# yzhang511/multi_modal_foundation_model

Hardware: NVIDIA B200
Metric: train trials/sec fwd+bwd (higher is better)
Workload: dtype bf16

## Files before the change

multi_modal_foundation_model_b200/csrc/common.cuh:

```cuda
#pragma once
#include <cuda.h>
#include <cuda_bf16.h>
#include <cuda_runtime.h>
#include <stdint.h>
#include <stdio.h>

namespace mmfm {

typedef __nv_bfloat16 bf16;

#define MMFM_DEVINL __device__ __forceinline__

MMFM_DEVINL uint32_t smem_u32(const void* p) { return (uint32_t)__cvta_generic_to_shared(p); }

MMFM_DEVINL bool elect_one() {
  uint32_t pred = 0;
  asm volatile(
      "{\n\t.reg .pred P1;\n\t.reg .b32 R1;\n\t"
      "elect.sync R1|P1, 0xffffffff;\n\t"
      "selp.u32 %0, 1, 0, P1;\n\t}\n"
      : "=r"(pred));
  return pred != 0;
}

// ... 37 lines not shown
      : "memory");
#else
  asm volatile(
      "{\n\t.reg .pred p;\n\t"
      "mbarrier.try_wait.parity.shared::cta.b64 p, [%1], %2;\n\t"
      "selp.u32 %0, 1, 0, p;\n\t}\n"
      : "=r"(ok)
      : "r"(smem_u32(bar)), "r"(parity)
      : "memory");
#endif
  return ok != 0;
}
MMFM_DEVINL void mbar_wait(uint64_t* bar, uint32_t parity) {
  if (mbar_try_wait(bar, parity)) return;
  uint32_t n = 0;
  while (!mbar_try_wait(bar, parity)) {
    if (++n > MMFM_MBAR_SPIN_LIMIT) {
      printf("mmfm: mbarrier wait timeout block(%d,%d,%d) thread %d parity %u bar %u\n", blockIdx.x, blockIdx.y,
             blockIdx.z, threadIdx.x, parity, smem_u32(bar));
      __trap();
    }
  }
}
MMFM_DEVINL void mbar_wait_relaxed(uint64_t* bar, uint32_t parity) {
  if (mbar_try_wait(bar, parity)) return;
  uint32_t n = 0;
  while (!mbar_try_wait(bar, parity)) {
    __nanosleep(40);
    if (++n > MMFM_MBAR_SPIN_LIMIT) {
      printf("mmfm: mbarrier wait timeout block(%d,%d,%d) thread %d parity %u bar %u\n", blockIdx.x, blockIdx.y,
             blockIdx.z, threadIdx.x, parity, smem_u32(bar));
      __trap();
    }
  }
}

MMFM_DEVINL void tma_prefetch_desc(const CUtensorMap* m) {
  asm volatile("prefetch.tensormap [%0];" ::"l"(m) : "memory");
}
MMFM_DEVINL void tma_load_2d_addr(uint32_t smem_dst, const CUtensorMap* m, uint64_t* bar, int c0, int c1) {
  asm volatile(
      "cp.async.bulk.tensor.2d.shared::cluster.global.mbarrier::complete_tx::bytes [%0], [%1, {%3, %4}], [%2];"
      ::"r"(smem_dst), "l"(m), "r"(smem_u32(bar)), "r"(c0), "r"(c1)
      : "memory");
}

MMFM_DEVINL void tma_store_2d(const CUtensorMap* m, uint32_t smem_src, int c0, int c1) {
  asm volatile("cp.async.bulk.tensor.2d.global.shared::cta.bulk_group [%0, {%2, %3}], [%1];" ::"l"(m), "r"(smem_src),
               "r"(c0), "r"(c1)
               : "memory");
}
MMFM_DEVINL void tma_store_3d(const CUtensorMap* m, uint32_t smem_src, int c0, int c1, int c2) {
  asm volatile("cp.async.bulk.tensor.3d.global.shared::cta.bulk_group [%0, {%2, %3, %4}], [%1];" ::"l"(m), "r"(smem_src),
               "r"(c0), "r"(c1), "r"(c2)
               : "memory");
}
MMFM_DEVINL void bulk_commit_group() { asm volatile("cp.async.bulk.commit_group;" ::: "memory"); }
template <int N>
MMFM_DEVINL void bulk_wait_group_read() {
  asm volatile("cp.async.bulk.wait_group.read %0;" ::"n"(N) : "memory");
}
template <int N>
MMFM_DEVINL void bulk_wait_group() {
  asm volatile("cp.async.bulk.wait_group %0;" ::"n"(N) : "memory");
}

MMFM_DEVINL void tma_load_2d_mc(uint32_t smem_dst, const CUtensorMap* m, uint64_t* bar, int c0, int c1, uint16_t mask) {
  asm volatile(
      "cp.async.bulk.tensor.2d.shared::cluster.global.mbarrier::complete_tx::bytes.multicast::cluster [%0], [%1, {%3, %4}], [%2], %5;"
      ::"r"(smem_dst), "l"(m), "r"(smem_u32(bar)), "r"(c0), "r"(c1), "h"(mask)
      : "memory");
}
MMFM_DEVINL void umma_commit_mc(uint64_t* bar, uint16_t mask) {
  asm volatile("tcgen05.commit.cta_group::1.mbarrier::arrive::one.shared::cluster.multicast::cluster.b64 [%0], %1;" ::"r"(
                   smem_u32(bar)),
               "h"(mask)
               : "memory");
}
MMFM_DEVINL uint32_t cluster_ctarank() {
  uint32_t r;
  asm volatile("mov.u32 %0, %%cluster_ctarank;" : "=r"(r));
  return r;
}
MMFM_DEVINL void cluster_sync_all() {
  asm volatile("barrier.cluster.arrive.release.aligned;\n\tbarrier.cluster.wait.acquire.aligned;" ::: "memory");
}

MMFM_DEVINL void tma_prefetch_l2_2d(const CUtensorMap* m, int c0, int c1) {
  asm volatile("cp.async.bulk.prefetch.tensor.2d.L2.global.tile [%0, {%1, %2}];" ::"l"(m), "r"(c0), "r"(c1) : "memory");
}

MMFM_DEVINL void tmem_alloc(uint32_t* smem_slot, uint32_t ncols) {
  asm volatile("tcgen05.alloc.cta_group::1.sync.aligned.shared::cta.b32 [%0], %1;" ::"r"(smem_u32(smem_slot)),
               "r"(ncols)
               : "memory");
}
MMFM_DEVINL void tmem_relinquish() {
  asm volatile("tcgen05.relinquish_alloc_permit.cta_group::1.sync.aligned;" ::: "memory");
}
MMFM_DEVINL void tmem_dealloc(uint32_t taddr, uint32_t ncols) {
  asm volatile("tcgen05.dealloc.cta_group::1.sync.aligned.b32 %0, %1;" ::"r"(taddr), "r"(ncols) : "memory");
}
MMFM_DEVINL void tc_fence_before() { asm volatile("tcgen05.fence::before_thread_sync;" ::: "memory"); }
MMFM_DEVINL void tc_fence_after() { asm volatile("tcgen05.fence::after_thread_sync;" ::: "memory"); }

MMFM_DEVINL void umma_bf16(uint32_t tmem_d, uint64_t desc_a, uint64_t desc_b, uint32_t idesc, uint32_t accumulate) {
  asm volatile(
      "{\n\t.reg .pred p;\n\t"
      "setp.ne.b32 p, %4, 0;\n\t"
      "tcgen05.mma.cta_group::1.kind::f16 [%0], %1, %2, %3, p;\n\t}\n" ::"r"(tmem_d),
      "l"(desc_a), "l"(desc_b), "r"(idesc), "r"(accumulate)
      : "memory");
}
MMFM_DEVINL void umma_bf16_ts(uint32_t tmem_d, uint32_t tmem_a, uint64_t desc_b, uint32_t idesc, uint32_t accumulate) {
  asm volatile(
      "{\n\t.reg .pred p;\n\t"
      "setp.ne.b32 p, %4, 0;\n\t"
      "tcgen05.mma.cta_group::1.kind::f16 [%0], [%1], %2, %3, p;\n\t}\n" ::"r"(tmem_d),
      "r"(tmem_a), "l"(desc_b), "r"(idesc), "r"(accumulate)
      : "memory");
}
MMFM_DEVINL void umma_commit(uint64_t* bar) {
  asm volatile("tcgen05.commit.cta_group::1.mbarrier::arrive::one.shared::cluster.b64 [%0];" ::"r"(smem_u32(bar))
               : "memory");
}

MMFM_DEVINL void tmem_ld32(uint32_t taddr, uint32_t (&r)[32]) {
  asm volatile(
      "tcgen05.ld.sync.aligned.32x32b.x32.b32 "
      "{%0, %1, %2, %3, %4, %5, %6, %7, %8, %9, %10, %11, %12, %13, %14, %15, "
      "%16, %17, %18, %19, %20, %21, %22, %23, %24, %25, %26, %27, %28, %29, %30, %31}, [%32];"
      : "=r"(r[0]), "=r"(r[1]), "=r"(r[2]), "=r"(r[3]), "=r"(r[4]), "=r"(r[5]), "=r"(r[6]), "=r"(r[7]),
        "=r"(r[8]), "=r"(r[9]), "=r"(r[10]), "=r"(r[11]), "=r"(r[12]), "=r"(r[13]), "=r"(r[14]), "=r"(r[15]),
        "=r"(r[16]), "=r"(r[17]), "=r"(r[18]), "=r"(r[19]), "=r"(r[20]), "=r"(r[21]), "=r"(r[22]),
        "=r"(r[23]), "=r"(r[24]), "=r"(r[25]), "=r"(r[26]), "=r"(r[27]), "=r"(r[28]), "=r"(r[29]),
        "=r"(r[30]), "=r"(r[31])
      : "r"(taddr)
      : "memory");
}
MMFM_DEVINL void tmem_ld16(uint32_t taddr, uint32_t (&r)[16]) {
  asm volatile(
      "tcgen05.ld.sync.aligned.32x32b.x16.b32 "
      "{%0, %1, %2, %3, %4, %5, %6, %7, %8, %9, %10, %11, %12, %13, %14, %15}, [%16];"
      : "=r"(r[0]), "=r"(r[1]), "=r"(r[2]), "=r"(r[3]), "=r"(r[4]), "=r"(r[5]), "=r"(r[6]), "=r"(r[7]),
        "=r"(r[8]), "=r"(r[9]), "=r"(r[10]), "=r"(r[11]), "=r"(r[12]), "=r"(r[13]), "=r"(r[14]), "=r"(r[15])
      : "r"(taddr)
      : "memory");
}
MMFM_DEVINL void tmem_ld_wait() { asm volatile("tcgen05.wait::ld.sync.aligned;" ::: "memory"); }
MMFM_DEVINL void tmem_st16(uint32_t taddr, const uint32_t (&r)[16]) {
  asm volatile(
      "tcgen05.st.sync.aligned.32x32b.x16.b32 [%0], "
      "{%1, %2, %3, %4, %5, %6, %7, %8, %9, %10, %11, %12, %13, %14, %15, %16};" ::"r"(taddr),
      "r"(r[0]), "r"(r[1]), "r"(r[2]), "r"(r[3]), "r"(r[4]), "r"(r[5]), "r"(r[6]), "r"(r[7]), "r"(r[8]), "r"(r[9]),
      "r"(r[10]), "r"(r[11]), "r"(r[12]), "r"(r[13]), "r"(r[14]), "r"(r[15])
      : "memory");
}
MMFM_DEVINL void tmem_st8(uint32_t taddr, const uint32_t (&r)[8]) {
  asm volatile("tcgen05.st.sync.aligned.32x32b.x8.b32 [%0], {%1, %2, %3, %4, %5, %6, %7, %8};" ::"r"(taddr), "r"(r[0]),
               "r"(r[1]), "r"(r[2]), "r"(r[3]), "r"(r[4]), "r"(r[5]), "r"(r[6]), "r"(r[7])
               : "memory");
}
MMFM_DEVINL void tmem_st_wait() { asm volatile("tcgen05.wait::st.sync.aligned;" ::: "memory"); }

MMFM_DEVINL uint64_t make_smem_desc(uint32_t saddr, uint32_t lbo_bytes, uint32_t sbo_bytes, uint32_t layout) {
  uint64_t d = 0;
  d |= (uint64_t)((saddr >> 4) & 0x3FFF);
  d |= (uint64_t)((lbo_bytes >> 4) & 0x3FFF) << 16;
  d |= (uint64_t)((sbo_bytes >> 4) & 0x3FFF) << 32;
  d |= (uint64_t)1 << 46;
  d |= (uint64_t)(layout & 7) << 61;
  return d;
}
__host__ __device__ inline uint32_t make_idesc_bf16(uint32_t M, uint32_t N, uint32_t a_mn, uint32_t b_mn) {
  uint32_t d = 0;
  d |= 1u << 4;
  d |= 1u << 7;
  d |= 1u << 10;
  d |= (a_mn & 1u) << 15;
  d |= (b_mn & 1u) << 16;
  d |= ((N >> 3) & 0x3F) << 17;
  d |= ((M >> 4) & 0x1F) << 24;
  return d;
}

constexpr int kPhiloxRounds = 7;

MMFM_DEVINL void mulhilo32(uint32_t a, uint32_t b, uint32_t& hi, uint32_t& lo) {
  const unsigned long long p = (unsigned long long)a * (unsigned long long)b;
  hi = (uint32_t)(p >> 32);
  lo = (uint32_t)p;
}

MMFM_DEVINL uint4 philox4x32(uint32_t c0, uint32_t c1, uint32_t c2, uint32_t c3, uint32_t k0, uint32_t k1) {
#pragma unroll
  for (int r = 0; r < kPhiloxRounds; ++r) {
    uint32_t hi0, lo0, hi1, lo1;
    mulhilo32(0xD2511F53u, c0, hi0, lo0);
    mulhilo32(0xCD9E8D57u, c2, hi1, lo1);
    const uint32_t n0 = hi1 ^ c1 ^ k0;
    const uint32_t n2 = hi0 ^ c3 ^ k1;
    c0 = n0; c1 = lo1; c2 = n2; c3 = lo0;
    k0 += 0x9E3779B9u; k1 += 0xBB67AE85u;
  }
  return make_uint4(c0, c1, c2, c3);
}
// ... 224 lines not shown
```

multi_modal_foundation_model_b200/csrc/gemm_ts.cu:

```cuda
#include "common.cuh"
#include <stdlib.h>
#include "host_util.h"
#include "../../include/mmfm_b200.h"

#ifdef MMFM_DBG_TIMING
__device__ long long g_dbg_ts[8][64];
__device__ __forceinline__ long long dbg_now() {
  long long t;
  asm volatile("mov.u64 %0, %%globaltimer;" : "=l"(t) :: "memory");
  return t;
}
#define DBG_TS(role, slot) do { if (blockIdx.x == 5 && (slot) < 64) g_dbg_ts[role][slot] = dbg_now(); } while (0)
__device__ long long g_dbg_cta[160][2];
extern "C" int mmfm_debug_read_gemm_ts(long long* out) {
  return (int)cudaMemcpyFromSymbol(out, g_dbg_ts, sizeof(long long) * 8 * 64);
}
extern "C" int mmfm_debug_read_gemm_cta(long long* out) {
  return (int)cudaMemcpyFromSymbol(out, g_dbg_cta, sizeof(long long) * 160 * 2);
}
#else
#define DBG_TS(role, slot) do { } while (0)
#endif

namespace mmfm {

constexpr int kTsBM = 128, kTsBK = 64;
constexpr int kTsEpiWarps = 16, kTsFirstEpi = 4;
constexpr int kTsThreads = (kTsFirstEpi + kTsEpiWarps) * 32;

enum TsEpi : int {
  TS_BF16 = 0,
  TS_SOFTSIGN = 1,
  TS_F32 = 2,
  TS_RES = 3,
  TS_GELU_DG = 4,
  TS_MULAUX = 5,
  TS_DSOFTSIGN = 6,
  TS_ROWDOT = 7
};

template <int EPI>
struct TsCfg {
  static constexpr bool kF32 = EPI == TS_F32 || EPI == TS_RES;
  static constexpr bool kHasIn = EPI == TS_RES || EPI == TS_MULAUX || EPI == TS_DSOFTSIGN || EPI == TS_ROWDOT;
  static constexpr bool kTwoOut = EPI == TS_GELU_DG;
  static constexpr uint32_t kRowBytes = kF32 ? 128u : 64u;
  static constexpr uint32_t kSlice = 128u * kRowBytes;
  static constexpr uint32_t kOut = 4u * kSlice;
  static constexpr uint32_t kBuf = kOut * (kTwoOut ? 2u : 1u);
};
constexpr int kTsMaxStages = 6;
constexpr size_t kTsMaxSmem = 230400;

template <int EPI, int BN>
__global__ void __launch_bounds__(kTsThreads, 1) gemm_tn_ts_kernel(const __grid_constant__ CUtensorMap tmA,
                                                                    const __grid_constant__ CUtensorMap tmB,
                                                                    const __grid_constant__ CUtensorMap tmD,
                                                                    const __grid_constant__ CUtensorMap tmD2,
                                                                    const __grid_constant__ CUtensorMap tmIn,
                                                                    const mmfm_gemm_args p, int tiles_n, int n_tiles,
                                                                    int bstat, int nst) {
  using Cfg = TsCfg<EPI>;
  constexpr int STAGES = kTsMaxStages;
  constexpr uint32_t kABytes = kTsBM * kTsBK * 2, kBBytes = BN * kTsBK * 2;
  constexpr uint32_t kTsStageBytes = kABytes + kBBytes;
  constexpr int NU = BN / 128;
  constexpr int kTsBN = BN;
  extern __shared__ uint8_t smem_raw[];
  __shared__ __align__(8) uint64_t full_bar[STAGES], empty_bar[STAGES];
  __shared__ __align__(8) uint64_t acc_full[2], acc_empty[2], in_full[2], stg_full[2], stg_free[2], b_full;
  __shared__ uint32_t tmem_slot;

  const int warp = threadIdx.x >> 5, lane = threadIdx.x & 31;
  const int nkb = (p.K + kTsBK - 1) / kTsBK;
  if (threadIdx.x == 0) DBG_TS(7, 63);
#ifdef MMFM_DBG_TIMING
  if (threadIdx.x == 0 && blockIdx.x < 160) g_dbg_cta[blockIdx.x][0] = dbg_now();
#endif
  const uint32_t smem_base = (smem_u32(smem_raw) + 1023u) & ~1023u;
  uint8_t* smem_al = smem_raw + (smem_base - smem_u32(smem_raw));
  const uint32_t b_res = bstat ? (uint32_t)nkb * kBBytes : 0u;
  const uint32_t st_bytes = bstat ? kABytes : kTsStageBytes;
  const uint32_t ring_base = smem_base + b_res;
  const uint32_t stg_off = b_res + (uint32_t)nst * st_bytes;
  const uint32_t stg_base = smem_base + stg_off;
  uint8_t* stg_ptr = smem_al + stg_off;

  pdl_trigger();
  if (warp == 0 && lane == 0) {
    tma_prefetch_desc(&tmA);
    tma_prefetch_desc(&tmB);
    tma_prefetch_desc(&tmD);
    if (Cfg::kTwoOut) tma_prefetch_desc(&tmD2);
    if (Cfg::kHasIn) tma_prefetch_desc(&tmIn);
#pragma unroll
    for (int s = 0; s < STAGES; ++s) {
      mbar_init(&full_bar[s], 1);
      mbar_init(&empty_bar[s], 1);
    }
#pragma unroll
    for (int i = 0; i < 2; ++i) {
      mbar_init(&acc_full[i], 1);
      mbar_init(&acc_empty[i], kTsEpiWarps);
      mbar_init(&in_full[i], 1);
      mbar_init(&stg_full[i], kTsEpiWarps);
      mbar_init(&stg_free[i], 1);
    }
    mbar_init(&b_full, 1);
    fence_mbar_init();
  }
  if (warp == 1) {
    tmem_alloc(&tmem_slot, 2u * BN);
    tmem_relinquish();
  }
  tc_fence_before();
  __syncthreads();
  tc_fence_after();
  const uint32_t tmem_base = tmem_slot;
  pdl_wait();

  if (warp == 0) {
    if (elect_one()) {
      uint32_t it = 0;
      const uint32_t ns = (uint32_t)nst;
      if (bstat) {
        const int n0 = ((int)blockIdx.x % tiles_n) * kTsBN;
        mbar_arrive_expect_tx(&b_full, b_res);
        for (int kb = 0; kb < nkb; ++kb) tma_load_2d_addr(smem_base + kb * kBBytes, &tmB, &b_full, kb * kTsBK, n0);
      }
      for (int tile = blockIdx.x; tile < n_tiles; tile += gridDim.x) {
        const int m0 = (tile / tiles_n) * kTsBM, n0 = (tile % tiles_n) * kTsBN;
        for (int kb = 0; kb < nkb; ++kb, ++it) {
          const uint32_t s = it % ns;
          if (it >= ns) mbar_wait(&empty_bar[s], ((it / ns) - 1) & 1);
          mbar_arrive_expect_tx(&full_bar[s], st_bytes);
          const uint32_t a_dst = ring_base + s * st_bytes;
          tma_load_2d_addr(a_dst, &tmA, &full_bar[s], kb * kTsBK, m0);
          if (!bstat) tma_load_2d_addr(a_dst + kABytes, &tmB, &full_bar[s], kb * kTsBK, n0);
        }
        DBG_TS(0, (int)(it / (uint32_t)nkb) - 1);
      }
    }
  } else if (warp == 1) {
    if (elect_one()) {
      const uint32_t idesc = make_idesc_bf16(kTsBM, kTsBN, 0, 0);
      uint32_t it = 0, t = 0;
      const uint32_t ns = (uint32_t)nst;
      if (bstat) mbar_wait(&b_full, 0);
      for (int tile = blockIdx.x; tile < n_tiles; tile += gridDim.x, ++t) {
        const uint32_t buf = t & 1u;
        if (t >= 2) mbar_wait(&acc_empty[buf], ((t >> 1) - 1) & 1);
        tc_fence_after();
        const uint32_t d_tmem = tmem_base + buf * kTsBN;
        for (int kb = 0; kb < nkb; ++kb, ++it) {
          const uint32_t s = it % ns;
          mbar_wait(&full_bar[s], (it / ns) & 1);
          tc_fence_after();
          const uint32_t a_addr = ring_base + s * st_bytes;
          const uint32_t b_addr = bstat ? smem_base + kb * kBBytes : a_addr + kABytes;
#pragma unroll
          for (int k = 0; k < kTsBK / 16; ++k)
            umma_bf16(d_tmem, make_smem_desc(a_addr + k * 32, 16, 1024, 2), make_smem_desc(b_addr + k * 32, 16, 1024, 2),
                      idesc, (kb > 0 || k > 0) ? 1u : 0u);
          umma_commit(&empty_bar[s]);
          if (kb == 0) DBG_TS(1, (int)t);
        }
        umma_commit(&acc_full[buf]);
        DBG_TS(2, (int)t);
      }
    }
  } else if (warp == 2) {
    if (elect_one()) {
      uint32_t u = 0;
      for (int tile = blockIdx.x; tile < n_tiles; tile += gridDim.x) {
        const int m0 = (tile / tiles_n) * kTsBM, n0 = (tile % tiles_n) * kTsBN;
#pragma unroll 1
        for (int hh = 0; hh < NU; ++hh, ++u) {
          const uint32_t sb = u & 1u;
          mbar_wait(&stg_full[sb], (u >> 1) & 1);
          DBG_TS(3, (int)u);
          const uint32_t src = stg_base + sb * Cfg::kBuf;
          const int nu = n0 + 128 * hh;
#pragma unroll
          for (int h = 0; h < 4; ++h) {
            if (nu + 32 * h < p.N) {
              tma_store_2d(&tmD, src + h * Cfg::kSlice, nu + 32 * h, m0);
              if (Cfg::kTwoOut) tma_store_2d(&tmD2, src + Cfg::kOut + h * Cfg::kSlice, nu + 32 * h, m0);
            }
          }
          bulk_commit_group();
          bulk_wait_group_read<0>();
          DBG_TS(4, (int)u);
          mbar_arrive(&stg_free[sb]);
        }
      }
      bulk_wait_group<0>();
    }
  } else if (warp == 3) {
    if (Cfg::kHasIn && elect_one()) {
      uint32_t u = 0;
      for (int tile = blockIdx.x; tile < n_tiles; tile += gridDim.x) {
        const int m0 = (tile / tiles_n) * kTsBM, n0 = (tile % tiles_n) * kTsBN;
#pragma unroll 1
        for (int hh = 0; hh < NU; ++hh, ++u) {
          const uint32_t sb = u & 1u;
          const int nu = n0 + 128 * hh;
          if (nu >= p.N) {
            if (u >= 2) mbar_wait(&stg_free[sb], ((u >> 1) - 1) & 1);
            mbar_arrive(&in_full[sb]);
            continue;
          }
          if (u >= 2) mbar_wait(&stg_free[sb], ((u >> 1) - 1) & 1);
          int nbox = (p.N - nu + 31) / 32;
          if (nbox > 4) nbox = 4;
          mbar_arrive_expect_tx(&in_full[sb], (uint32_t)nbox * Cfg::kSlice);
          DBG_TS(5, (int)u);
          const uint32_t dst = stg_base + sb * Cfg::kBuf;
          for (int h = 0; h < nbox; ++h) tma_load_2d_addr(dst + h * Cfg::kSlice, &tmIn, &in_full[sb], nu + 32 * h, m0);
        }
      }
    }
  } else {
    const int ew = warp - kTsFirstEpi;
    const int quad = warp & 3, h = ew >> 2;
    const int row = quad * 32 + lane;
    bool drop = false;
    unsigned long long seed = 0ull;
    if (EPI == TS_RES || EPI == TS_ROWDOT) {
      drop = p.drop.thresh != 0u;
      if (drop) seed = *p.drop.seed;
    }
    const uint32_t drop_gpr = (uint32_t)((p.N + 15) >> 4);
    const float act_scale = p.act_scale, inv_scale = 1.0f / p.act_scale;
    const uint32_t row_off = (uint32_t)row * Cfg::kRowBytes;
    const uint32_t swz = Cfg::kF32 ? (uint32_t)(row & 7) : (uint32_t)((row >> 1) & 3);

    uint32_t t = 0, u = 0;
    for (int tile = blockIdx.x; tile < n_tiles; tile += gridDim.x, ++t) {
      const uint32_t buf = t & 1u;
      const int m0 = (tile / tiles_n) * kTsBM, n0 = (tile % tiles_n) * kTsBN;
      mbar_wait(&acc_full[buf], (t >> 1) & 1);
      tc_fence_after();
#pragma unroll 1
      for (int hh = 0; hh < NU; ++hh, ++u) {
      const uint32_t sb = u & 1u;
      const int nb = n0 + 128 * hh + 32 * h;
      const bool has_cols = nb < p.N;
      if (Cfg::kHasIn) mbar_wait(&in_full[sb], (u >> 1) & 1);
      else if (u >= 2) mbar_wait(&stg_free[sb], ((u >> 1) - 1) & 1);
      if (warp == kTsFirstEpi && lane == 0) DBG_TS(6, (int)u);
      if (has_cols) {
        uint8_t* box = stg_ptr + sb * Cfg::kBuf + h * Cfg::kSlice + row_off;
        const uint32_t t_row = tmem_base + buf * kTsBN + ((uint32_t)(quad * 32) << 16) + (uint32_t)(128 * hh + 32 * h);
        const long long r = (long long)m0 + row;
        float dot = 0.f;
#pragma unroll
        for (int c0 = 0; c0 < 32; c0 += 16) {
          uint32_t acc[16];
          tmem_ld16(t_row + (uint32_t)c0, acc);
          tmem_ld_wait();
          float v[16];
          if (p.bias) {
            if (nb + c0 + 16 <= p.N) {
#pragma unroll
              for (int j4 = 0; j4 < 4; ++j4) {
                const float4 b4 = __ldg(reinterpret_cast<const float4*>(p.bias + nb + c0) + j4);
                v[4 * j4 + 0] = __uint_as_float(acc[4 * j4 + 0]) + b4.x;
                v[4 * j4 + 1] = __uint_as_float(acc[4 * j4 + 1]) + b4.y;
                v[4 * j4 + 2] = __uint_as_float(acc[4 * j4 + 2]) + b4.z;
                v[4 * j4 + 3] = __uint_as_float(acc[4 * j4 + 3]) + b4.w;
              }
            } else {
#pragma unroll
              for (int j = 0; j < 16; ++j)
                v[j] = __uint_as_float(acc[j]) + ((nb + c0 + j < p.N) ? __ldg(p.bias + nb + c0 + j) : 0.f);
            }
          } else {
#pragma unroll
            for (int j = 0; j < 16; ++j) v[j] = __uint_as_float(acc[j]);
          }
          if (EPI == TS_RES) {
            if (drop) {
              const uint4 w = drop_bytes16(seed, p.drop.site, (uint64_t)r, drop_gpr, (uint32_t)((nb + c0) >> 4));
#pragma unroll
              for (int j = 0; j < 16; ++j) v[j] = (drop_byte(w, j) < p.drop.thresh) ? 0.f : v[j] * p.drop.scale;
            }
#pragma unroll
            for (int j4 = 0; j4 < 4; ++j4) {
              float4* q = reinterpret_cast<float4*>(box + ((((uint32_t)(c0 >> 2) + j4) ^ swz) << 4));
              const float4 rv = *q;
              *q = make_float4(v[4 * j4] + rv.x, v[4 * j4 + 1] + rv.y, v[4 * j4 + 2] + rv.z, v[4 * j4 + 3] + rv.w);
            }
          } else if (EPI == TS_F32) {
#pragma unroll
            for (int j4 = 0; j4 < 4; ++j4)
              *reinterpret_cast<float4*>(box + ((((uint32_t)(c0 >> 2) + j4) ^ swz) << 4)) =
                  make_float4(v[4 * j4], v[4 * j4 + 1], v[4 * j4 + 2], v[4 * j4 + 3]);
          } else {
            if (EPI == TS_SOFTSIGN) {
#pragma unroll
              for (int j = 0; j < 16; ++j) v[j] = softsign(v[j]) * act_scale;
            }
            float d2[16];
            if (EPI == TS_GELU_DG) {
#pragma unroll
              for (int j = 0; j < 16; j += 2) gelu_erf_both2(v[j], v[j + 1], v[j], v[j + 1], d2[j], d2[j + 1]);
            }
            uint4 wdrop = make_uint4(0u, 0u, 0u, 0u);
            if (EPI == TS_ROWDOT && drop)
              wdrop = drop_bytes16(seed, p.drop.site, (uint64_t)r, drop_gpr, (uint32_t)((nb + c0) >> 4));
#pragma unroll
            for (int q8 = 0; q8 < 2; ++q8) {
              uint4* q = reinterpret_cast<uint4*>(box + ((((uint32_t)(c0 >> 3) + q8) ^ swz) << 4));
              if (EPI == TS_ROWDOT) {
                const uint4 a4 = *q;
                const uint32_t aw[4] = {a4.x, a4.y, a4.z, a4.w};
#pragma unroll
                for (int e = 0; e < 4; ++e) {
                  const float2 a2 = unpack_bf16x2(aw[e]);
                  dot = fmaf(v[8 * q8 + 2 * e], a2.x, dot);
                  dot = fmaf(v[8 * q8 + 2 * e + 1], a2.y, dot);
                }
                if (drop) {
#pragma unroll
                  for (int e = 0; e < 8; ++e)
                    v[8 * q8 + e] = (drop_byte(wdrop, 8 * q8 + e) < p.drop.thresh) ? 0.f : v[8 * q8 + e] * p.drop.scale;
                }
              }
              if (EPI == TS_MULAUX || EPI == TS_DSOFTSIGN) {
                const uint4 a4 = *q;
                const uint32_t aw[4] = {a4.x, a4.y, a4.z, a4.w};
#pragma unroll
                for (int e = 0; e < 4; ++e) {
                  const float2 a2 = unpack_bf16x2(aw[e]);
                  float f0 = a2.x, f1 = a2.y;
                  if (EPI == TS_DSOFTSIGN) {
                    const float t0 = 1.0f - fabsf(f0 * inv_scale), t1 = 1.0f - fabsf(f1 * inv_scale);
                    f0 = act_scale * t0 * t0;
                    f1 = act_scale * t1 * t1;
                  }
                  v[8 * q8 + 2 * e] *= f0;
                  v[8 * q8 + 2 * e + 1] *= f1;
                }
              }
              *q = make_uint4(pack_bf16x2(v[8 * q8], v[8 * q8 + 1]), pack_bf16x2(v[8 * q8 + 2], v[8 * q8 + 3]),
                              pack_bf16x2(v[8 * q8 + 4], v[8 * q8 + 5]), pack_bf16x2(v[8 * q8 + 6], v[8 * q8 + 7]));
              if (EPI == TS_GELU_DG)
                *reinterpret_cast<uint4*>(box + Cfg::kOut + ((((uint32_t)(c0 >> 3) + q8) ^ swz) << 4)) =
                    make_uint4(pack_bf16x2(d2[8 * q8], d2[8 * q8 + 1]), pack_bf16x2(d2[8 * q8 + 2], d2[8 * q8 + 3]),
                               pack_bf16x2(d2[8 * q8 + 4], d2[8 * q8 + 5]), pack_bf16x2(d2[8 * q8 + 6], d2[8 * q8 + 7]));
            }
          }
        }
        if (EPI == TS_ROWDOT && r < p.M) {
          const long long bb = r / p.rowdot_S;
          const int ii = (int)(r - bb * p.rowdot_S);
          p.rowdot[(bb * (p.N >> 5) + (nb >> 5)) * p.rowdot_S + ii] = dot;
        }
      }
      tc_fence_before();
      fence_proxy_async();
      __syncwarp();
      if (lane == 0) {
        if (hh == NU - 1) mbar_arrive(&acc_empty[buf]);
        mbar_arrive(&stg_full[sb]);
        if (warp == kTsFirstEpi) DBG_TS(7, (int)u);
      }
      }
    }
  }
  tc_fence_before();
  __syncthreads();
  if (threadIdx.x == 0) DBG_TS(7, 62);
#ifdef MMFM_DBG_TIMING
  if (threadIdx.x == 0 && blockIdx.x < 160) { __threadfence(); g_dbg_cta[blockIdx.x][1] = dbg_now(); }
#endif
  if (warp == 1) tmem_dealloc(tmem_base, 2u * BN);
}

}

using namespace mmfm;

template <int EPI, int BN>
static int launch_ts_bn(const mmfm_gemm_args* a, cudaStream_t st) {
  using Cfg = TsCfg<EPI>;
  CUtensorMap tmA, tmB, tmD, tmD2, tmIn;
  memset(&tmD2, 0, sizeof(tmD2));
  memset(&tmIn, 0, sizeof(tmIn));
  int rc = make_tmap_bf16_2d(&tmA, a->A, (uint64_t)a->M, (uint64_t)a->K, (uint64_t)a->lda, kTsBK, kTsBM, TMA_SW_128);
  if (rc) return rc;
  rc = make_tmap_bf16_2d(&tmB, a->B, (uint64_t)a->N, (uint64_t)a->K, (uint64_t)a->ldb, kTsBK, BN, TMA_SW_128);
  if (rc) return rc;
  if (Cfg::kF32) rc = make_tmap_f32_2d(&tmD, a->D, (uint64_t)a->M, (uint64_t)a->N, (uint64_t)a->ldd, 32, 128, TMA_SW_128);
  else rc = make_tmap_bf16_2d(&tmD, a->D, (uint64_t)a->M, (uint64_t)a->N, (uint64_t)a->ldd, 32, 128, TMA_SW_64);
  if (rc) return rc;
  if (Cfg::kTwoOut) {
    rc = make_tmap_bf16_2d(&tmD2, a->D2, (uint64_t)a->M, (uint64_t)a->N, (uint64_t)a->ldd, 32, 128, TMA_SW_64);
    if (rc) return rc;
  }
  if (EPI == TS_RES) rc = make_tmap_f32_2d(&tmIn, a->res, (uint64_t)a->M, (uint64_t)a->N, (uint64_t)a->ldr, 32, 128, TMA_SW_128);
  else if (Cfg::kHasIn) rc = make_tmap_bf16_2d(&tmIn, a->aux, (uint64_t)a->M, (uint64_t)a->N, (uint64_t)a->ldaux, 32, 128, TMA_SW_64);
  if (rc) return rc;
  static bool attr_set = false;
  if (!attr_set) {
    MMFM_CHECK_CUDA(cudaFuncSetAttribute(gemm_tn_ts_kernel<EPI, BN>, cudaFuncAttributeMaxDynamicSharedMemorySize, (int)kTsMaxSmem));
    attr_set = true;
  }
  const int tiles_n = (a->N + BN - 1) / BN, tiles_m = (a->M + kTsBM - 1) / kTsBM;
  const int n_tiles = tiles_n * tiles_m;
  const int sms = device_sm_count();
  int grid = n_tiles < sms ? n_tiles : sms;
  const size_t a_stage = (size_t)kTsBM * kTsBK * 2, b_stage = (size_t)BN * kTsBK * 2;
  size_t room = (kTsMaxSmem - 1024 - 2 * (size_t)Cfg::kBuf) / (a_stage + b_stage);
  int nst = room > 4 ? 4 : (int)room, bstat = 0;
  size_t smem = 1024 + (size_t)nst * (a_stage + b_stage) + 2 * (size_t)Cfg::kBuf;
  static int bstat_env = -1;
  if (bstat_env < 0) {
    const char* e = getenv("MMFM_GEMM_TS_BSTAT");
    bstat_env = (e && e[0] == '1') ? 1 : 0;
  }
  const int nkb = (a->K + kTsBK - 1) / kTsBK;
  const size_t b_res = (size_t)nkb * b_stage;
  if (bstat_env && tiles_n <= sms && tiles_m >= 2 * (sms / tiles_n) &&
      1024 + b_res + 2 * a_stage + 2 * (size_t)Cfg::kBuf <= kTsMaxSmem) {
    room = (kTsMaxSmem - 1024 - b_res - 2 * (size_t)Cfg::kBuf) / a_stage;
    nst = room > (size_t)kTsMaxStages ? kTsMaxStages : (int)room;
    bstat = 1;
    grid = (sms / tiles_n) * tiles_n;
    smem = 1024 + b_res + (size_t)nst * a_stage + 2 * (size_t)Cfg::kBuf;
  }
  set_l2_window(a->D, (size_t)a->M * (size_t)a->ldd * (a->d_fp32 ? 4 : 2));
  MMFM_CHECK_CUDA(launch_pdl(gemm_tn_ts_kernel<EPI, BN>, dim3(grid), dim3(kTsThreads), smem, st, tmA, tmB, tmD, tmD2, tmIn, *a,
                             tiles_n, n_tiles, bstat, nst));
  return 0;
}

template <int EPI>
static int launch_ts(const mmfm_gemm_args* a, cudaStream_t st) {
  static int bn_env = -1;
  if (bn_env < 0) {
    const char* e = getenv("MMFM_GEMM_TS_BN");
    bn_env = e ? atoi(e) : 256;
  }
  if (bn_env == 256 && a->N % 256 == 0) return launch_ts_bn<EPI, 256>(a, st);
  return launch_ts_bn<EPI, 128>(a, st);
}

namespace mmfm {

static bool al16(const void* p) { return (reinterpret_cast<uintptr_t>(p) & 15) == 0; }

int try_launch_gemm_ts(const mmfm_gemm_args* a, cudaStream_t st) {
  static int enabled = -1;
  if (enabled < 0) {
    const char* e = getenv("MMFM_GEMM_TS");
    enabled = (e && e[0] == '0') ? 0 : 1;
  }
  if (!enabled) return 0;
  if (a->N <= 64 || a->N % 4 != 0 || a->remap_T > 0 || a->row_zero != nullptr) return 0;
  const bool f32 = a->d_fp32 != 0;
  const int esz = f32 ? 4 : 2;
  if (!al16(a->D) || (a->ldd * esz) % 16 != 0) return 0;
  if (a->bias && !al16(a->bias)) return 0;
  const bool drop = a->drop.thresh != 0;
  int epi = -1;
  if (a->res) {
    static int res_env = -1;
    if (res_env < 0) {
      const char* e = getenv("MMFM_GEMM_TS_RES");
      res_env = (e && e[0] == '1') ? 1 : 0;
    }
    if (!res_env) return 0;
    if (a->act != MMFM_ACT_NONE || !f32 || a->D2 || !al16(a->res) || (a->ldr * 4) % 16 != 0) return 0;
    epi = TS_RES;
  } else {
    if (drop && a->act != MMFM_ACT_ROWDOT_DROP) return 0;
    switch (a->act) {
      case MMFM_ACT_NONE:
        if (a->D2) return 0;
        epi = f32 ? TS_F32 : TS_BF16;
        break;
      case MMFM_ACT_SOFTSIGN:
        if (f32 || a->D2) return 0;
        epi = TS_SOFTSIGN;
        break;
      case MMFM_ACT_GELU_DG:
        if (f32 || !a->D2 || !al16(a->D2)) return 0;
        epi = TS_GELU_DG;
        break;
      case MMFM_ACT_MULAUX:
      case MMFM_ACT_DSOFTSIGN:
        if (f32 || a->D2 || !a->aux || !al16(a->aux) || (a->ldaux * 2) % 16 != 0) return 0;
        epi = a->act == MMFM_ACT_MULAUX ? TS_MULAUX : TS_DSOFTSIGN;
        break;
      case MMFM_ACT_ROWDOT_DROP:
        if (f32 || a->D2 || a->bias || !a->aux || !al16(a->aux) || (a->ldaux * 2) % 16 != 0 || a->N % 32 != 0 || !a->rowdot)
          return 0;
        epi = TS_ROWDOT;
        break;
      default:
        return 0;
    }
  }
  int rc = 0;
  switch (epi) {
    case TS_BF16: rc = launch_ts<TS_BF16>(a, st); break;
    case TS_SOFTSIGN: rc = launch_ts<TS_SOFTSIGN>(a, st); break;
    case TS_F32: rc = launch_ts<TS_F32>(a, st); break;
    case TS_RES: rc = launch_ts<TS_RES>(a, st); break;
    case TS_GELU_DG: rc = launch_ts<TS_GELU_DG>(a, st); break;
    case TS_MULAUX: rc = launch_ts<TS_MULAUX>(a, st); break;
    case TS_DSOFTSIGN: rc = launch_ts<TS_DSOFTSIGN>(a, st); break;
    case TS_ROWDOT: rc = launch_ts<TS_ROWDOT>(a, st); break;
    default: return 0;
  }
  return rc == 0 ? 1 : rc;
}

}
```

multi_modal_foundation_model_b200/csrc/host_util.h:

```cpp
#pragma once
#include <cuda.h>
#include <cuda_runtime.h>
#include <stdint.h>
#include <stdio.h>
#include <string.h>

namespace mmfm {

void set_error(const char* fmt, ...);
const char* get_error();

#define MMFM_CHECK_CUDA(expr)                                                              \
  do {                                                                                     \
    cudaError_t _e = (expr);                                                               \
    if (_e != cudaSuccess) {                                                               \
      ::mmfm::set_error("%s:%d: %s -> %s", __FILE__, __LINE__, #expr, cudaGetErrorString(_e)); \
      return -2;                                                                           \
    }                                                                                      \
  } while (0)

#define MMFM_REQUIRE(cond, ...)            \
  do {                                     \
    if (!(cond)) {                         \
      ::mmfm::set_error(__VA_ARGS__);      \
      return -1;                           \
    }                                      \
  } while (0)

enum TmaSwizzle { TMA_SW_NONE = 0, TMA_SW_32 = 1, TMA_SW_64 = 2, TMA_SW_128 = 3 };

int make_tmap_bf16_2d(CUtensorMap* out, const void* base, uint64_t rows, uint64_t cols, uint64_t ld,
                      uint32_t box_cols, uint32_t box_rows, TmaSwizzle swz);

int make_tmap_f32_2d(CUtensorMap* out, const void* base, uint64_t rows, uint64_t cols, uint64_t ld, uint32_t box_cols,
                     uint32_t box_rows, TmaSwizzle swz);

int make_tmap_bf16_3d(CUtensorMap* out, const void* base, uint64_t batch, uint64_t rows, uint64_t cols, uint64_t ld,
                      uint32_t box_cols, uint32_t box_rows, TmaSwizzle swz);

int device_sm_count();

struct DetNeed {
  long long bytes;
  int tickets;
};
bool det_need_gemm(int kind, long long d0, long long d1, long long d2, DetNeed* need);
bool det_need_norm(int kind, long long d0, long long d1, long long d2, DetNeed* need);
bool det_need_glue(int kind, long long d0, long long d1, long long d2, DetNeed* need);
int det_ws_check(const void* buf, long long bytes, const unsigned int* tickets, int n_tickets, const DetNeed& need,
                 const char* who);

bool pdl_enabled();

void set_l2_window(const void* ptr, size_t bytes);
bool take_l2_window(cudaAccessPolicyWindow* w);

template <typename... KArgs, typename... Args>
inline cudaError_t launch_pdl(void (*kernel)(KArgs...), dim3 grid, dim3 block, size_t smem, cudaStream_t st, Args... args) {
  cudaLaunchConfig_t cfg = {};
  cfg.gridDim = grid;
  cfg.blockDim = block;
  cfg.dynamicSmemBytes = smem;
  cfg.stream = st;
  cudaLaunchAttribute attr[2];
  attr[0].id = cudaLaunchAttributeProgrammaticStreamSerialization;
  attr[0].val.programmaticStreamSerializationAllowed = pdl_enabled() ? 1 : 0;
  cfg.attrs = attr;
  cfg.numAttrs = 1;
  if (take_l2_window(&attr[1].val.accessPolicyWindow)) {
    attr[1].id = cudaLaunchAttributeAccessPolicyWindow;
    cfg.numAttrs = 2;
  }
  return cudaLaunchKernelEx(&cfg, kernel, KArgs(args)...);
}

}
```

Before: 26590.

## Use 2-CTA cluster UMMA for the BN=256 TS GEMM path

Replaces the single-CTA 128x256 tile kernel with a 2-CTA cluster variant that issues cta_group::2 tcgen05.mma over a 256x256 tile. Each CTA loads half of A and half of B into its own shared memory, which halves per-CTA B traffic and shared memory per stage and allows a deeper ring. It also removes the optional B-resident (bstat) mode and sizes the grid from the occupancy of active clusters. This adds cross-CTA mbarrier traffic, cluster syncs and a drain loop at the end, and any error in the paired-CTA protocol can hang or corrupt results.

```diff
diff --git a/multi_modal_foundation_model_b200/csrc/common.cuh b/multi_modal_foundation_model_b200/csrc/common.cuh
--- a/multi_modal_foundation_model_b200/csrc/common.cuh
+++ b/multi_modal_foundation_model_b200/csrc/common.cuh
@@ -143,6 +143,20 @@
   asm volatile("mov.u32 %0, %%cluster_ctarank;" : "=r"(r));
   return r;
 }
+MMFM_DEVINL uint32_t mapa_shared(uint32_t addr, uint32_t rank) {
+  uint32_t r;
+  asm volatile("mapa.shared::cluster.u32 %0, %1, %2;" : "=r"(r) : "r"(addr), "r"(rank));
+  return r;
+}
+MMFM_DEVINL void mbar_arrive_cluster(uint32_t bar_cluster) {
+  asm volatile("mbarrier.arrive.release.cluster.shared::cluster.b64 _, [%0];" ::"r"(bar_cluster) : "memory");
+}
+MMFM_DEVINL void tma_load_2d_2cta(uint32_t smem_dst, const CUtensorMap* m, uint32_t bar_cluster, int c0, int c1) {
+  asm volatile(
+      "cp.async.bulk.tensor.2d.cta_group::2.shared::cluster.global.mbarrier::complete_tx::bytes [%0], [%1, {%3, %4}], [%2];"
+      ::"r"(smem_dst), "l"(m), "r"(bar_cluster), "r"(c0), "r"(c1)
+      : "memory");
+}
 MMFM_DEVINL void cluster_sync_all() {
   asm volatile("barrier.cluster.arrive.release.aligned;\n\tbarrier.cluster.wait.acquire.aligned;" ::: "memory");
 }
@@ -161,6 +175,17 @@
 }
 MMFM_DEVINL void tmem_dealloc(uint32_t taddr, uint32_t ncols) {
   asm volatile("tcgen05.dealloc.cta_group::1.sync.aligned.b32 %0, %1;" ::"r"(taddr), "r"(ncols) : "memory");
+}
+MMFM_DEVINL void tmem_alloc_2cta(uint32_t* smem_slot, uint32_t ncols) {
+  asm volatile("tcgen05.alloc.cta_group::2.sync.aligned.shared::cta.b32 [%0], %1;" ::"r"(smem_u32(smem_slot)),
+               "r"(ncols)
+               : "memory");
+}
+MMFM_DEVINL void tmem_relinquish_2cta() {
+  asm volatile("tcgen05.relinquish_alloc_permit.cta_group::2.sync.aligned;" ::: "memory");
+}
+MMFM_DEVINL void tmem_dealloc_2cta(uint32_t taddr, uint32_t ncols) {
+  asm volatile("tcgen05.dealloc.cta_group::2.sync.aligned.b32 %0, %1;" ::"r"(taddr), "r"(ncols) : "memory");
 }
 MMFM_DEVINL void tc_fence_before() { asm volatile("tcgen05.fence::before_thread_sync;" ::: "memory"); }
 MMFM_DEVINL void tc_fence_after() { asm volatile("tcgen05.fence::after_thread_sync;" ::: "memory"); }
@@ -183,6 +208,20 @@
 }
 MMFM_DEVINL void umma_commit(uint64_t* bar) {
   asm volatile("tcgen05.commit.cta_group::1.mbarrier::arrive::one.shared::cluster.b64 [%0];" ::"r"(smem_u32(bar))
+               : "memory");
+}
+MMFM_DEVINL void umma_bf16_2cta(uint32_t tmem_d, uint64_t desc_a, uint64_t desc_b, uint32_t idesc, uint32_t accumulate) {
+  asm volatile(
+      "{\n\t.reg .pred p;\n\t"
+      "setp.ne.b32 p, %4, 0;\n\t"
+      "tcgen05.mma.cta_group::2.kind::f16 [%0], %1, %2, %3, p;\n\t}\n" ::"r"(tmem_d),
+      "l"(desc_a), "l"(desc_b), "r"(idesc), "r"(accumulate)
+      : "memory");
+}
+MMFM_DEVINL void umma_commit_2cta_mc(uint64_t* bar, uint16_t mask) {
+  asm volatile("tcgen05.commit.cta_group::2.mbarrier::arrive::one.shared::cluster.multicast::cluster.b64 [%0], %1;" ::"r"(
+                   smem_u32(bar)),
+               "h"(mask)
                : "memory");
 }
 
diff --git a/multi_modal_foundation_model_b200/csrc/gemm_ts.cu b/multi_modal_foundation_model_b200/csrc/gemm_ts.cu
--- a/multi_modal_foundation_model_b200/csrc/gemm_ts.cu
+++ b/multi_modal_foundation_model_b200/csrc/gemm_ts.cu
@@ -51,38 +51,38 @@
 };
 constexpr int kTsMaxStages = 6;
 constexpr size_t kTsMaxSmem = 230400;
-
-template <int EPI, int BN>
+constexpr uint32_t kTsABytes = kTsBM * kTsBK * 2, kTsStageBytes = 2 * kTsABytes;
+
+template <int EPI, int CG>
 __global__ void __launch_bounds__(kTsThreads, 1) gemm_tn_ts_kernel(const __grid_constant__ CUtensorMap tmA,
                                                                     const __grid_constant__ CUtensorMap tmB,
                                                                     const __grid_constant__ CUtensorMap tmD,
                                                                     const __grid_constant__ CUtensorMap tmD2,
                                                                     const __grid_constant__ CUtensorMap tmIn,
                                                                     const mmfm_gemm_args p, int tiles_n, int n_tiles,
-                                                                    int bstat, int nst) {
+                                                                    int nst) {
+  static_assert(CG == 1 || CG == 2, "one CTA or a pair");
   using Cfg = TsCfg<EPI>;
   constexpr int STAGES = kTsMaxStages;
-  constexpr uint32_t kABytes = kTsBM * kTsBK * 2, kBBytes = BN * kTsBK * 2;
-  constexpr uint32_t kTsStageBytes = kABytes + kBBytes;
-  constexpr int NU = BN / 128;
-  constexpr int kTsBN = BN;
+  constexpr int kTsBN = 128 * CG;
+  constexpr int NU = kTsBN / 128;
   extern __shared__ uint8_t smem_raw[];
   __shared__ __align__(8) uint64_t full_bar[STAGES], empty_bar[STAGES];
-  __shared__ __align__(8) uint64_t acc_full[2], acc_empty[2], in_full[2], stg_full[2], stg_free[2], b_full;
+  __shared__ __align__(8) uint64_t acc_full[2], acc_empty[2], in_full[2], stg_full[2], stg_free[2];
   __shared__ uint32_t tmem_slot;
 
   const int warp = threadIdx.x >> 5, lane = threadIdx.x & 31;
   const int nkb = (p.K + kTsBK - 1) / kTsBK;
+  const uint32_t rank = CG == 2 ? cluster_ctarank() : 0u;
+  const int tile0 = (int)blockIdx.x / CG, tile_step = (int)gridDim.x / CG;
   if (threadIdx.x == 0) DBG_TS(7, 63);
 #ifdef MMFM_DBG_TIMING
   if (threadIdx.x == 0 && blockIdx.x < 160) g_dbg_cta[blockIdx.x][0] = dbg_now();
 #endif
   const uint32_t smem_base = (smem_u32(smem_raw) + 1023u) & ~1023u;
   uint8_t* smem_al = smem_raw + (smem_base - smem_u32(smem_raw));
-  const uint32_t b_res = bstat ? (uint32_t)nkb * kBBytes : 0u;
-  const uint32_t st_bytes = bstat ? kABytes : kTsStageBytes;
-  const uint32_t ring_base = smem_base + b_res;
-  const uint32_t stg_off = b_res + (uint32_t)nst * st_bytes;
+  const uint32_t ring_base = smem_base;
+  const uint32_t stg_off = (uint32_t)nst * kTsStageBytes;
   const uint32_t stg_base = smem_base + stg_off;
   uint8_t* stg_ptr = smem_al + stg_off;
 
@@ -101,20 +101,25 @@
 #pragma unroll
     for (int i = 0; i < 2; ++i) {
       mbar_init(&acc_full[i], 1);
-      mbar_init(&acc_empty[i], kTsEpiWarps);
+      mbar_init(&acc_empty[i], kTsEpiWarps * CG);
       mbar_init(&in_full[i], 1);
       mbar_init(&stg_full[i], kTsEpiWarps);
       mbar_init(&stg_free[i], 1);
     }
-    mbar_init(&b_full, 1);
     fence_mbar_init();
   }
   if (warp == 1) {
-    tmem_alloc(&tmem_slot, 2u * BN);
-    tmem_relinquish();
+    if (CG == 2) {
+      tmem_alloc_2cta(&tmem_slot, 2u * kTsBN);
+      tmem_relinquish_2cta();
+    } else {
+      tmem_alloc(&tmem_slot, 2u * kTsBN);
+      tmem_relinquish();
+    }
   }
   tc_fence_before();
   __syncthreads();
+  if (CG == 2) cluster_sync_all();
   tc_fence_after();
   const uint32_t tmem_base = tmem_slot;
   pdl_wait();
@@ -123,31 +128,37 @@
     if (elect_one()) {
       uint32_t it = 0;
       const uint32_t ns = (uint32_t)nst;
-      if (bstat) {
-        const int n0 = ((int)blockIdx.x % tiles_n) * kTsBN;
-        mbar_arrive_expect_tx(&b_full, b_res);
-        for (int kb = 0; kb < nkb; ++kb) tma_load_2d_addr(smem_base + kb * kBBytes, &tmB, &b_full, kb * kTsBK, n0);
-      }
-      for (int tile = blockIdx.x; tile < n_tiles; tile += gridDim.x) {
-        const int m0 = (tile / tiles_n) * kTsBM, n0 = (tile % tiles_n) * kTsBN;
+      const uint32_t full_lead = CG == 2 ? mapa_shared(smem_u32(&full_bar[0]), 0) : 0u;
+      for (int tile = tile0; tile < n_tiles; tile += tile_step) {
+        const int m0 = (tile / tiles_n) * (kTsBM * CG) + kTsBM * (int)rank;
+        const int nb0 = (tile % tiles_n) * kTsBN + 128 * (int)rank;
         for (int kb = 0; kb < nkb; ++kb, ++it) {
           const uint32_t s = it % ns;
           if (it >= ns) mbar_wait(&empty_bar[s], ((it / ns) - 1) & 1);
-          mbar_arrive_expect_tx(&full_bar[s], st_bytes);
-          const uint32_t a_dst = ring_base + s * st_bytes;
-          tma_load_2d_addr(a_dst, &tmA, &full_bar[s], kb * kTsBK, m0);
-          if (!bstat) tma_load_2d_addr(a_dst + kABytes, &tmB, &full_bar[s], kb * kTsBK, n0);
+          const uint32_t a_dst = ring_base + s * kTsStageBytes;
+          if (CG == 2) {
+            if (rank == 0) mbar_arrive_expect_tx(&full_bar[s], 2u * kTsStageBytes);
+            const uint32_t fb = full_lead + s * (uint32_t)sizeof(uint64_t);
+            tma_load_2d_2cta(a_dst, &tmA, fb, kb * kTsBK, m0);
+            tma_load_2d_2cta(a_dst + kTsABytes, &tmB, fb, kb * kTsBK, nb0);
+          } else {
+            mbar_arrive_expect_tx(&full_bar[s], kTsStageBytes);
+            tma_load_2d_addr(a_dst, &tmA, &full_bar[s], kb * kTsBK, m0);
+            tma_load_2d_addr(a_dst + kTsABytes, &tmB, &full_bar[s], kb * kTsBK, nb0);
+          }
         }
         DBG_TS(0, (int)(it / (uint32_t)nkb) - 1);
       }
+      if (CG == 2) {
+        for (uint32_t j = it > ns ? it - ns : 0u; j < it; ++j) mbar_wait(&empty_bar[j % ns], (j / ns) & 1);
+      }
     }
   } else if (warp == 1) {
-    if (elect_one()) {
-      const uint32_t idesc = make_idesc_bf16(kTsBM, kTsBN, 0, 0);
+    if (rank == 0 && elect_one()) {
+      const uint32_t idesc = make_idesc_bf16(kTsBM * CG, kTsBN, 0, 0);
       uint32_t it = 0, t = 0;
       const uint32_t ns = (uint32_t)nst;
-      if (bstat) mbar_wait(&b_full, 0);
-      for (int tile = blockIdx.x; tile < n_tiles; tile += gridDim.x, ++t) {
+      for (int tile = tile0; tile < n_tiles; tile += tile_step, ++t) {
         const uint32_t buf = t & 1u;
         if (t >= 2) mbar_wait(&acc_empty[buf], ((t >> 1) - 1) & 1);
         tc_fence_after();
@@ -156,24 +167,29 @@
           const uint32_t s = it % ns;
           mbar_wait(&full_bar[s], (it / ns) & 1);
           tc_fence_after();
-          const uint32_t a_addr = ring_base + s * st_bytes;
-          const uint32_t b_addr = bstat ? smem_base + kb * kBBytes : a_addr + kABytes;
-#pragma unroll
-          for (int k = 0; k < kTsBK / 16; ++k)
-            umma_bf16(d_tmem, make_smem_desc(a_addr + k * 32, 16, 1024, 2), make_smem_desc(b_addr + k * 32, 16, 1024, 2),
-                      idesc, (kb > 0 || k > 0) ? 1u : 0u);
-          umma_commit(&empty_bar[s]);
+          const uint32_t a_addr = ring_base + s * kTsStageBytes;
+          const uint32_t b_addr = a_addr + kTsABytes;
+#pragma unroll
+          for (int k = 0; k < kTsBK / 16; ++k) {
+            const uint64_t da = make_smem_desc(a_addr + k * 32, 16, 1024, 2), db = make_smem_desc(b_addr + k * 32, 16, 1024, 2);
+            const uint32_t acc = (kb > 0 || k > 0) ? 1u : 0u;
+            if (CG == 2) umma_bf16_2cta(d_tmem, da, db, idesc, acc);
+            else umma_bf16(d_tmem, da, db, idesc, acc);
+          }
+          if (CG == 2) umma_commit_2cta_mc(&empty_bar[s], 0x3);
+          else umma_commit(&empty_bar[s]);
           if (kb == 0) DBG_TS(1, (int)t);
         }
-        umma_commit(&acc_full[buf]);
+        if (CG == 2) umma_commit_2cta_mc(&acc_full[buf], 0x3);
+        else umma_commit(&acc_full[buf]);
         DBG_TS(2, (int)t);
       }
     }
   } else if (warp == 2) {
     if (elect_one()) {
       uint32_t u = 0;
-      for (int tile = blockIdx.x; tile < n_tiles; tile += gridDim.x) {
-        const int m0 = (tile / tiles_n) * kTsBM, n0 = (tile % tiles_n) * kTsBN;
+      for (int tile = tile0; tile < n_tiles; tile += tile_step) {
+        const int m0 = (tile / tiles_n) * (kTsBM * CG) + kTsBM * (int)rank, n0 = (tile % tiles_n) * kTsBN;
 #pragma unroll 1
         for (int hh = 0; hh < NU; ++hh, ++u) {
           const uint32_t sb = u & 1u;
@@ -199,8 +215,8 @@
   } else if (warp == 3) {
     if (Cfg::kHasIn && elect_one()) {
       uint32_t u = 0;
-      for (int tile = blockIdx.x; tile < n_tiles; tile += gridDim.x) {
-        const int m0 = (tile / tiles_n) * kTsBM, n0 = (tile % tiles_n) * kTsBN;
+      for (int tile = tile0; tile < n_tiles; tile += tile_step) {
+        const int m0 = (tile / tiles_n) * (kTsBM * CG) + kTsBM * (int)rank, n0 = (tile % tiles_n) * kTsBN;
 #pragma unroll 1
         for (int hh = 0; hh < NU; ++hh, ++u) {
           const uint32_t sb = u & 1u;
@@ -234,11 +250,12 @@
     const float act_scale = p.act_scale, inv_scale = 1.0f / p.act_scale;
     const uint32_t row_off = (uint32_t)row * Cfg::kRowBytes;
     const uint32_t swz = Cfg::kF32 ? (uint32_t)(row & 7) : (uint32_t)((row >> 1) & 3);
+    const uint32_t acc_empty_addr = CG == 2 ? mapa_shared(smem_u32(&acc_empty[0]), 0) : smem_u32(&acc_empty[0]);
 
     uint32_t t = 0, u = 0;
-    for (int tile = blockIdx.x; tile < n_tiles; tile += gridDim.x, ++t) {
+    for (int tile = tile0; tile < n_tiles; tile += tile_step, ++t) {
       const uint32_t buf = t & 1u;
-      const int m0 = (tile / tiles_n) * kTsBM, n0 = (tile % tiles_n) * kTsBN;
+      const int m0 = (tile / tiles_n) * (kTsBM * CG) + kTsBM * (int)rank, n0 = (tile % tiles_n) * kTsBN;
       mbar_wait(&acc_full[buf], (t >> 1) & 1);
       tc_fence_after();
 #pragma unroll 1
@@ -362,7 +379,10 @@
       fence_proxy_async();
       __syncwarp();
       if (lane == 0) {
-        if (hh == NU - 1) mbar_arrive(&acc_empty[buf]);
+        if (hh == NU - 1) {
+          if (CG == 2) mbar_arrive_cluster(acc_empty_addr + buf * (uint32_t)sizeof(uint64_t));
+          else mbar_arrive(&acc_empty[buf]);
+        }
         mbar_arrive(&stg_full[sb]);
         if (warp == kTsFirstEpi) DBG_TS(7, (int)u);
       }
@@ -371,26 +391,32 @@
   }
   tc_fence_before();
   __syncthreads();
+  if (CG == 2) cluster_sync_all();
   if (threadIdx.x == 0) DBG_TS(7, 62);
 #ifdef MMFM_DBG_TIMING
   if (threadIdx.x == 0 && blockIdx.x < 160) { __threadfence(); g_dbg_cta[blockIdx.x][1] = dbg_now(); }
 #endif
-  if (warp == 1) tmem_dealloc(tmem_base, 2u * BN);
+  if (warp == 1) {
+    tc_fence_after();
+    if (CG == 2) tmem_dealloc_2cta(tmem_base, 2u * kTsBN);
+    else tmem_dealloc(tmem_base, 2u * kTsBN);
+  }
 }
 
 }
 
 using namespace mmfm;
 
-template <int EPI, int BN>
-static int launch_ts_bn(const mmfm_gemm_args* a, cudaStream_t st) {
+template <int EPI, int CG>
+static int launch_ts_cg(const mmfm_gemm_args* a, cudaStream_t st) {
   using Cfg = TsCfg<EPI>;
+  constexpr int BN = 128 * CG, BM = kTsBM * CG;
   CUtensorMap tmA, tmB, tmD, tmD2, tmIn;
   memset(&tmD2, 0, sizeof(tmD2));
   memset(&tmIn, 0, sizeof(tmIn));
   int rc = make_tmap_bf16_2d(&tmA, a->A, (uint64_t)a->M, (uint64_t)a->K, (uint64_t)a->lda, kTsBK, kTsBM, TMA_SW_128);
   if (rc) return rc;
-  rc = make_tmap_bf16_2d(&tmB, a->B, (uint64_t)a->N, (uint64_t)a->K, (uint64_t)a->ldb, kTsBK, BN, TMA_SW_128);
+  rc = make_tmap_bf16_2d(&tmB, a->B, (uint64_t)a->N, (uint64_t)a->K, (uint64_t)a->ldb, kTsBK, 128, TMA_SW_128);
   if (rc) return rc;
   if (Cfg::kF32) rc = make_tmap_f32_2d(&tmD, a->D, (uint64_t)a->M, (uint64_t)a->N, (uint64_t)a->ldd, 32, 128, TMA_SW_128);
   else rc = make_tmap_bf16_2d(&tmD, a->D, (uint64_t)a->M, (uint64_t)a->N, (uint64_t)a->ldd, 32, 128, TMA_SW_64);
@@ -402,37 +428,41 @@
   if (EPI == TS_RES) rc = make_tmap_f32_2d(&tmIn, a->res, (uint64_t)a->M, (uint64_t)a->N, (uint64_t)a->ldr, 32, 128, TMA_SW_128);
   else if (Cfg::kHasIn) rc = make_tmap_bf16_2d(&tmIn, a->aux, (uint64_t)a->M, (uint64_t)a->N, (uint64_t)a->ldaux, 32, 128, TMA_SW_64);
   if (rc) return rc;
-  static bool attr_set = false;
-  if (!attr_set) {
-    MMFM_CHECK_CUDA(cudaFuncSetAttribute(gemm_tn_ts_kernel<EPI, BN>, cudaFuncAttributeMaxDynamicSharedMemorySize, (int)kTsMaxSmem));
-    attr_set = true;
-  }
-  const int tiles_n = (a->N + BN - 1) / BN, tiles_m = (a->M + kTsBM - 1) / kTsBM;
+  constexpr size_t room = (kTsMaxSmem - 1024 - 2 * (size_t)Cfg::kBuf) / kTsStageBytes;
+  constexpr int kCap = CG == 2 ? kTsMaxStages : 4;
+  constexpr int nst = room > (size_t)kCap ? kCap : (int)room;
+  constexpr size_t smem = 1024 + (size_t)nst * kTsStageBytes + 2 * (size_t)Cfg::kBuf;
+  static_assert(nst >= 2, "ring too shallow");
+  auto kernel = gemm_tn_ts_kernel<EPI, CG>;
+  static int max_units = 0;
+  if (max_units == 0) {
+    MMFM_CHECK_CUDA(cudaFuncSetAttribute(kernel, cudaFuncAttributeMaxDynamicSharedMemorySize, (int)kTsMaxSmem));
+    if (CG == 1) {
+      max_units = device_sm_count();
+    } else {
+      cudaLaunchConfig_t cfg = {};
+      cfg.gridDim = dim3(2);
+      cfg.blockDim = dim3(kTsThreads);
+      cfg.dynamicSmemBytes = smem;
+      cudaLaunchAttribute attr;
+      attr.id = cudaLaunchAttributeClusterDimension;
+      attr.val.clusterDim.x = 2;
+      attr.val.clusterDim.y = 1;
+      attr.val.clusterDim.z = 1;
+      cfg.attrs = &attr;
+      cfg.numAttrs = 1;
+      int n = 0;
+      MMFM_CHECK_CUDA(cudaOccupancyMaxActiveClusters(&n, kernel, &cfg));
+      MMFM_REQUIRE(n > 0, "gemm_ts: no 2-CTA cluster of %zu bytes of shared memory fits", smem);
+      max_units = n;
+    }
+  }
+  const int tiles_n = (a->N + BN - 1) / BN, tiles_m = (a->M + BM - 1) / BM;
   const int n_tiles = tiles_n * tiles_m;
-  const int sms = device_sm_count();
-  int grid = n_tiles < sms ? n_tiles : sms;
-  const size_t a_stage = (size_t)kTsBM * kTsBK * 2, b_stage = (size_t)BN * kTsBK * 2;
-  size_t room = (kTsMaxSmem - 1024 - 2 * (size_t)Cfg::kBuf) / (a_stage + b_stage);
-  int nst = room > 4 ? 4 : (int)room, bstat = 0;
-  size_t smem = 1024 + (size_t)nst * (a_stage + b_stage) + 2 * (size_t)Cfg::kBuf;
-  static int bstat_env = -1;
-  if (bstat_env < 0) {
-    const char* e = getenv("MMFM_GEMM_TS_BSTAT");
-    bstat_env = (e && e[0] == '1') ? 1 : 0;
-  }
-  const int nkb = (a->K + kTsBK - 1) / kTsBK;
-  const size_t b_res = (size_t)nkb * b_stage;
-  if (bstat_env && tiles_n <= sms && tiles_m >= 2 * (sms / tiles_n) &&
-      1024 + b_res + 2 * a_stage + 2 * (size_t)Cfg::kBuf <= kTsMaxSmem) {
-    room = (kTsMaxSmem - 1024 - b_res - 2 * (size_t)Cfg::kBuf) / a_stage;
-    nst = room > (size_t)kTsMaxStages ? kTsMaxStages : (int)room;
-    bstat = 1;
-    grid = (sms / tiles_n) * tiles_n;
-    smem = 1024 + b_res + (size_t)nst * a_stage + 2 * (size_t)Cfg::kBuf;
-  }
+  const int units = n_tiles < max_units ? n_tiles : max_units;
   set_l2_window(a->D, (size_t)a->M * (size_t)a->ldd * (a->d_fp32 ? 4 : 2));
-  MMFM_CHECK_CUDA(launch_pdl(gemm_tn_ts_kernel<EPI, BN>, dim3(grid), dim3(kTsThreads), smem, st, tmA, tmB, tmD, tmD2, tmIn, *a,
-                             tiles_n, n_tiles, bstat, nst));
+  MMFM_CHECK_CUDA(launch_pdl_cluster(kernel, dim3(units * CG), dim3(kTsThreads), (unsigned)CG, smem, st, tmA, tmB, tmD,
+                                     tmD2, tmIn, *a, tiles_n, n_tiles, nst));
   return 0;
 }
 
@@ -443,8 +473,8 @@
     const char* e = getenv("MMFM_GEMM_TS_BN");
     bn_env = e ? atoi(e) : 256;
   }
-  if (bn_env == 256 && a->N % 256 == 0) return launch_ts_bn<EPI, 256>(a, st);
-  return launch_ts_bn<EPI, 128>(a, st);
+  if (bn_env == 256 && a->N % 256 == 0) return launch_ts_cg<EPI, 2>(a, st);
+  return launch_ts_cg<EPI, 1>(a, st);
 }
 
 namespace mmfm {
diff --git a/multi_modal_foundation_model_b200/csrc/host_util.h b/multi_modal_foundation_model_b200/csrc/host_util.h
--- a/multi_modal_foundation_model_b200/csrc/host_util.h
+++ b/multi_modal_foundation_model_b200/csrc/host_util.h
@@ -56,22 +56,31 @@
 bool take_l2_window(cudaAccessPolicyWindow* w);
 
 template <typename... KArgs, typename... Args>
-inline cudaError_t launch_pdl(void (*kernel)(KArgs...), dim3 grid, dim3 block, size_t smem, cudaStream_t st, Args... args) {
+inline cudaError_t launch_pdl_cluster(void (*kernel)(KArgs...), dim3 grid, dim3 block, unsigned cluster_x, size_t smem,
+                                      cudaStream_t st, Args... args) {
   cudaLaunchConfig_t cfg = {};
   cfg.gridDim = grid;
   cfg.blockDim = block;
   cfg.dynamicSmemBytes = smem;
   cfg.stream = st;
-  cudaLaunchAttribute attr[2];
+  cudaLaunchAttribute attr[3];
   attr[0].id = cudaLaunchAttributeProgrammaticStreamSerialization;
   attr[0].val.programmaticStreamSerializationAllowed = pdl_enabled() ? 1 : 0;
   cfg.attrs = attr;
   cfg.numAttrs = 1;
-  if (take_l2_window(&attr[1].val.accessPolicyWindow)) {
-    attr[1].id = cudaLaunchAttributeAccessPolicyWindow;
-    cfg.numAttrs = 2;
+  if (take_l2_window(&attr[cfg.numAttrs].val.accessPolicyWindow)) attr[cfg.numAttrs++].id = cudaLaunchAttributeAccessPolicyWindow;
+  if (cluster_x > 1) {
+    attr[cfg.numAttrs].id = cudaLaunchAttributeClusterDimension;
+    attr[cfg.numAttrs].val.clusterDim.x = cluster_x;
+    attr[cfg.numAttrs].val.clusterDim.y = 1;
+    attr[cfg.numAttrs].val.clusterDim.z = 1;
+    cfg.numAttrs++;
   }
   return cudaLaunchKernelEx(&cfg, kernel, KArgs(args)...);
 }
+template <typename... KArgs, typename... Args>
+inline cudaError_t launch_pdl(void (*kernel)(KArgs...), dim3 grid, dim3 block, size_t smem, cudaStream_t st, Args... args) {
+  return launch_pdl_cluster(kernel, grid, block, 1u, smem, st, args...);
+}
 
 }
```

Result: slower. 26070 (median of 6 runs) (-2.0%).
